# HKU-BAL/MegaGTA

Hardware: AMD Instinct MI355X
Metric: HMM-scored node expansions/sec + SdBG-build Gk-mer/s, k=45, 100Mx150bp (higher is better)
Workload: dtype u32

## Files before the change

include/megagta_hip.h:

```cpp
#ifndef MEGAGTA_HIP_H_
#define MEGAGTA_HIP_H_
#include <stdint.h>
#ifdef __cplusplus
extern "C" {
#endif

#define MGTA_OK 0
#define MGTA_EINVAL (-1)
#define MGTA_EHIP (-2)
#define MGTA_ENOMEM (-3)
#define MGTA_EUNSUPPORTED (-4)
#define MGTA_ESINK (-5)
#define MGTA_EOVERFLOW (-6)
#define MGTA_EINTERNAL (-7)

#define MGTA_NUM_BUCKETS 65536

typedef struct mgta_ctx mgta_ctx;
typedef struct mgta_reads mgta_reads;
typedef struct mgta_sdbg mgta_sdbg;
typedef struct mgta_hmm mgta_hmm;

const char *mgta_last_error(void);
const char *mgta_version(void);
// ... 28 lines not shown

typedef struct mgta_build_stats {
    int32_t k, words_per_key, words_per_tip, n_passes;
    int64_t n_reads, n_kmers;
    int64_t n_items;
    int64_t n_edges, n_tips, n_large;
    int64_t n_sort_launches;
    double ms_total;
    double ms_count, ms_gen, ms_sort, ms_emit, ms_d2h;
    double ms_sort_scatter;
    double ms_local_sort;
    int64_t n_big_segments;
    int64_t n_lsd_tiles;
    uint64_t bytes_peak;
    double ms_stage1;
} mgta_build_stats;

int mgta_reads_upload(mgta_ctx *, const uint32_t *packed_seq, uint64_t n_words, const uint64_t *start_idx,
                      uint64_t n_reads, mgta_reads **out);
int mgta_reads_adopt_device(mgta_ctx *, const uint32_t *d_packed_seq, uint64_t n_words,
                            const uint64_t *d_start_idx, uint64_t n_reads, mgta_reads **out);
void mgta_reads_free(mgta_reads *);

int mgta_sdbg_build_resident(mgta_ctx *, const mgta_reads *, uint64_t n_short_reads, int k, int min_count,
                             int need_mercy, int32_t bucket_begin, int32_t bucket_end ,
                             mgta_edge_sink sink, void *user, mgta_build_stats *stats);
int mgta_sdbg_last_counting(mgta_ctx *, int64_t *hist );
int mgta_sdbg_export_records_device(mgta_ctx *, void *d_dst, uint64_t capacity_bytes, uint64_t *n_records);
int mgta_sdbg_build(mgta_ctx *, const uint32_t *packed_seq, uint64_t n_words, const uint64_t *start_idx,
                    uint64_t n_reads, uint64_t n_short_reads, int k, int min_count, int need_mercy,
// ... 255 lines not shown
```

megagta_amd/_lib.py:

```python
from __future__ import annotations

import ctypes as C
import os

_HERE = os.path.dirname(os.path.abspath(__file__))
LIB_PATH = os.environ.get("MEGAGTA_HIP_LIB") or os.path.join(_HERE, "libmegagta_hip.so")


class MegaGtaError(RuntimeError):
    pass


class DenovoStats(C.Structure):
    _fields_ = [("n_tips", C.c_int64), ("n_bubbles", C.c_int64), ("n_bubble_candidates", C.c_int64), ("n_bubble_rounds", C.c_int64),
                ("n_paths", C.c_int64), ("n_unitig_sweeps", C.c_int64), ("n_contigs", C.c_int64), ("total_len", C.c_int64),
                ("ms_tips", C.c_float), ("ms_bubbles", C.c_float), ("ms_unitigs", C.c_float)]

    def as_dict(self):
        return {n: getattr(self, n) for n, _ in self._fields_}


class BuildStats(C.Structure):
    _fields_ = [("k", C.c_int32), ("words_per_key", C.c_int32), ("words_per_tip", C.c_int32), ("n_passes", C.c_int32),
                ("n_reads", C.c_int64), ("n_kmers", C.c_int64), ("n_items", C.c_int64), ("n_edges", C.c_int64),
                ("n_tips", C.c_int64), ("n_large", C.c_int64), ("n_sort_launches", C.c_int64), ("ms_total", C.c_double),
                ("ms_count", C.c_double), ("ms_gen", C.c_double), ("ms_sort", C.c_double), ("ms_emit", C.c_double),
                ("ms_d2h", C.c_double), ("ms_sort_scatter", C.c_double), ("ms_local_sort", C.c_double), ("n_big_segments", C.c_int64), ("n_lsd_tiles", C.c_int64),
                ("bytes_peak", C.c_uint64), ("ms_stage1", C.c_double)]

    def as_dict(self):
        return {n: getattr(self, n) for n, _ in self._fields_}


class AstarSide(C.Structure):
    _fields_ = [("ok", C.c_int32), ("fval", C.c_int32), ("length", C.c_int32), ("state_no", C.c_int32), ("state", C.c_int32),
                ("partial", C.c_int32), ("node_id", C.c_int64), ("n_closed", C.c_int64), ("n_expanded", C.c_int64),
                ("n_opened", C.c_int64), ("real_score", C.c_double), ("score", C.c_double)]


class AstarStats(C.Structure):
    _fields_ = [("n_seeds", C.c_int64), ("n_expansions", C.c_int64), ("n_opened", C.c_int64), ("n_retries", C.c_int64),
                ("ms_total", C.c_double), ("ms_kernel", C.c_double), ("n_grown", C.c_int64), ("n_rehash", C.c_int64),
                ("n_recycled", C.c_int64), ("pool_bytes", C.c_uint64), ("pool_used", C.c_uint64), ("n_resumes", C.c_int64),
# ... 228 lines not shown
```

megagta_amd/csrc/common.hpp:

```cpp
#pragma once
#include <hip/hip_runtime.h>

#include <cstdarg>
#include <cstdint>
#include <cstdio>
#include <cstring>
#include <exception>
#include <new>
#include <string>
#include <vector>

#include "../../include/megagta_hip.h"

namespace mgta {

void set_error(const char *fmt, ...);

struct HipError {
    int code;
};

#define MGTA_HIP_CHECK(expr)                                                                        \
    do {                                                                                            \
        hipError_t e_ = (expr);                                                                     \
// ... 44 lines not shown
    Timer(Timer &&o) noexcept : a(o.a), b(o.b), st(o.st) { o.a = o.b = nullptr; }
    ~Timer() { if (a) (void)hipEventDestroy(a); if (b) (void)hipEventDestroy(b); }
    void start() { MGTA_HIP_CHECK(hipEventRecord(a, st)); }
    void end() { MGTA_HIP_CHECK(hipEventRecord(b, st)); }
    float ms() const { float t = 0; MGTA_HIP_CHECK(hipEventElapsedTime(&t, a, b)); return t; }
    double stop() {
        MGTA_HIP_CHECK(hipGetLastError());
        end();
        MGTA_HIP_CHECK(hipEventSynchronize(b));
        MGTA_HIP_CHECK(hipGetLastError());
        return ms();
    }
};

enum Slot { S_BLOCK_COUNT, S_BLOCK_BASE, S_SCAN_TMP, S_SMALL, S_KEYS_A, S_KEYS_B, S_HIST, S_TILE_HEADS, S_TILE_BASE, S_CNT, S_BASE,
            S_FIRST, S_OUT_REC, S_OUT_LARGE, S_OUT_TIPS, S_PLAN, S_BIG, S_LSD, S_MULTI_COUNT, S_POS2ID, S_SOLID, S_MERCY, S_EDGE_COUNT, S_SIDE, S_NUM };

}

namespace mgta {
struct AstarArenas {
    DevBuf pool, meta;
};
}

struct mgta_ctx {
    int refs = 1;
    int device = 0;
    hipStream_t stream = nullptr;
    uint64_t mem_limit = 0;
    int force_full_lsd = 0;
// ... 71 lines not shown
```

megagta_amd/csrc/sdbg_build.hip:

```cpp
#include <algorithm>
#include <cmath>
#include <cstdlib>
#include <memory>
#include <type_traits>

#include "common.hpp"
#include "device_utils.hpp"
#include "scan.hpp"

namespace mgta {

constexpr int kDollar = 4;

template <int W>
struct Key {
    uint32_t w[W];
};

template <int W>
__device__ __forceinline__ void shl_bits(uint32_t (&x)[W], int s) {
    if (s == 0) return;
    if (s == 32) {
#pragma unroll
        for (int j = 0; j < W - 1; ++j) x[j] = x[j + 1];
// ... 45 lines not shown
    int k;
    uint32_t b_lo, b_hi;
    uint32_t *block_count;
    const uint64_t *block_base;
    void *out;
    unsigned long long *n_kmers;
    const unsigned long long *is_solid;
    int num_k1_per_read;
    uint64_t n_short;
    unsigned long long *n_sentinel;
    uint32_t multi_width, multi_n;
    uint64_t multi_magic;
    uint8_t *side;
    int side_shift;
    uint32_t side_bias;
};
constexpr int kMaxCountRanges = 64;

template <int W>
__device__ __forceinline__ void keep_masks(int n, uint32_t (&m)[W]) {
#pragma unroll
    for (int j = 0; j < W; ++j) {
        const int lo = j * 16;
        m[j] = n <= lo ? 0u : (n < lo + 16 ? ~0u << (32 - 2 * (n - lo)) : ~0u);
    }
}

template <int W, bool WRITE>
__global__ __launch_bounds__(kScanBlock) void item_scan_kernel(ScanArgs a) {
    __shared__ uint32_t s_cursor;
    __shared__ uint32_t s_wave_cnt[kScanBlock / 64];
    __shared__ uint32_t s_range_cnt[kMaxCountRanges];
    const int k = a.k;
    const int lane = lane_id(), wv = wave_id();
    __shared__ uint64_t s_start[kReadsPerBlock + 1];
    const bool multi = !WRITE && a.multi_n > 0;
    const uint64_t multi_magic = a.multi_magic;
    const bool magic24 = multi_magic < (1u << 24);
    uint64_t r0 = (uint64_t)blockIdx.x * kReadsPerBlock;
    uint64_t r1 = r0 + kReadsPerBlock < a.n_reads ? r0 + kReadsPerBlock : a.n_reads;
    if (threadIdx.x == 0) s_cursor = 0;
    if (!WRITE && threadIdx.x < kMaxCountRanges) s_range_cnt[threadIdx.x] = 0;
    if (threadIdx.x <= r1 - r0) s_start[threadIdx.x] = a.start[r0 + threadIdx.x];
    __syncthreads();
    Key<W> *out = reinterpret_cast<Key<W> *>(a.out);
    uint64_t base = WRITE ? a.block_base[blockIdx.x] : 0;
    uint32_t my_count = 0;
    unsigned long long kmers = 0;
    const int pad_bits = 2 * (16 * W - (k + 1));
    const bool even = !((k + 1) & 1);
    const bool few = multi && a.multi_n <= 8;
    uint32_t acc[8] = {0, 0, 0, 0, 0, 0, 0, 0};
    uint32_t m_edge[W], m_k[W], m_k1[W];
    keep_masks<W>(k + 1, m_edge);
    keep_masks<W>(k, m_k);
    keep_masks<W>(k - 1, m_k1);
    const bool in_bounds = wave_uniform((s_start[r1 - r0] >> 4) + (uint64_t)(W + 1)) < a.n_words;

    auto positions = [&](bool active, uint64_t r, uint64_t s0, int p, int npos) {
        bool run_first = p == 0, run_last = p == npos - 1;
        if (active && a.is_solid && r < a.n_short) {
// ... 21 lines not shown
                for (int j = 0; j <= W; ++j) raw[j] = a.packed[wi + j];
            } else {
#pragma unroll
                for (int j = 0; j <= W; ++j) raw[j] = (wi + j < a.n_words) ? a.packed[wi + j] : 0u;
            }
#pragma unroll
            for (int j = 0; j < W; ++j) e[j] = (uint32_t)(((((uint64_t)raw[j]) << 32) | (uint64_t)raw[j + 1]) >> (32 - sh)) & m_edge[j];
#pragma unroll
            for (int j = 0; j < W; ++j) rc[j] = rev_chars(~e[W - 1 - j]);
            shl_bits<W>(rc, pad_bits);
            bool pal = even;
            if (even) {
#pragma unroll
                for (int j = 0; j < W; ++j) pal = pal && (e[j] == rc[j]);
            }
            auto push = [&](int t, const uint32_t (&src)[W], int from) {
                const uint32_t b = ((src[0] << (2 * from)) >> 16);
                if (b < a.b_lo || b >= a.b_hi) return;
                if (WRITE) mask |= 1u << t;
                else if (multi) {
                    const uint32_t x = b - a.b_lo;
                    uint32_t range;
                    if (magic24) asm("v_mul_hi_u32_u24 %0, %1, %2" : "=v"(range) : "v"(x), "v"((uint32_t)multi_magic));
                    else range = (uint32_t)(((uint64_t)x * multi_magic) >> 32);
                    if (few) fields += 1u << (4 * range);
                    else atomicAdd(&s_range_cnt[range], 1u);
                }
                ++cnt;
            };
            if (run_first) {
                push(0, e, 0);
                if (!pal) push(1, rc, 2);
            }
            push(2, e, 1);
            if (!pal) push(3, rc, 1);
            if (run_last) {
                push(4, e, 2);
                if (!pal) push(5, rc, 0);
            }
        }
        if (!WRITE) {
            my_count += (uint32_t)cnt;
            if (few) {
#pragma unroll
                for (int g = 0; g < 8; ++g)
                    if (g < (int)a.multi_n) acc[g] += (fields >> (4 * g)) & 15u;
            }
        } else {
            const uint32_t inc = wave_incl_scan((uint32_t)cnt);
            const uint32_t tot = __shfl(inc, 63, 64);
            if (tot) {
                uint32_t wbase = 0;
                if (lane == 0) wbase = atomicAdd(&s_cursor, tot);
                const uint64_t first = base + (uint64_t)wave_uniform(wbase);
                char *const wave_out = reinterpret_cast<char *>(out + first);
                uint8_t *const wave_side = a.side ? a.side + first : nullptr;
                uint32_t slot = inc - (uint32_t)cnt;
                auto put = [&](int t, const uint32_t (&src)[W], int from, const uint32_t (&keep)[W], uint32_t flags) {
                    if (!((mask >> t) & 1u)) return;
                    Key<W> key;
#pragma unroll
// ... 52 lines not shown
            for (int g = 0; g < 8; ++g) {
                if (g < (int)a.multi_n) {
                    const uint32_t t = wave_sum(acc[g]);
                    if (lane == 0 && t) atomicAdd(&s_range_cnt[g], t);
                }
            }
        }
        if (lane == 0) s_wave_cnt[wv] = my_count;
        __syncthreads();
        if (threadIdx.x == 0 && !multi) {
            uint32_t t = 0;
            for (int w = 0; w < kScanBlock / 64; ++w) t += s_wave_cnt[w];
            a.block_count[blockIdx.x] = t;
        }
        if (multi && threadIdx.x < a.multi_n) a.block_count[(uint64_t)threadIdx.x * gridDim.x + blockIdx.x] = s_range_cnt[threadIdx.x];
        if (lane == 0 && kmers && a.n_kmers) atomicAdd(a.n_kmers, kmers);
    }
}

template <int W>
__global__ __launch_bounds__(kScanBlock) void item_write_closed_kernel(ScanArgs a) {
    __shared__ uint32_t s_read_base[kReadsPerBlock];
    __shared__ uint64_t s_start[kReadsPerBlock + 1];
    const int k = a.k;
    const int lane = lane_id(), wv = wave_id();
    const uint64_t r0 = (uint64_t)blockIdx.x * kReadsPerBlock;
    const uint64_t r1 = r0 + kReadsPerBlock < a.n_reads ? r0 + kReadsPerBlock : a.n_reads;
    if (wv == 0) {
        const uint64_t st = r0 + lane <= r1 ? a.start[r0 + lane] : 0, st_next = r0 + lane < r1 ? a.start[r0 + lane + 1] : st;
        s_start[lane] = st;
// ... 116 lines not shown
    for (int i = 0; i < N; ++i) { lo[i] = 0; hi[i] = 0; }
#pragma unroll
    for (int j = 0; j < W; ++j) {
        if (j == wi) {
#pragma unroll
            for (int i = 0; i < N; ++i) {
                lo[i] = key[i].w[j] - (BIASED && j == 0 ? d.bias : 0u);
                hi[i] = j > 0 ? key[i].w[j - 1] - (BIASED && j == 1 ? d.bias : 0u) : 0u;
                asm volatile("" : "+v"(lo[i]), "+v"(hi[i]));
            }
        }
    }
    const uint32_t mask = (1u << d.bits) - 1u;
#pragma unroll
    for (int i = 0; i < N; ++i) dg[i] = __builtin_amdgcn_alignbit(hi[i], lo[i], (uint32_t)off) & mask;
}

__device__ __forceinline__ uint32_t xcd_tile(uint32_t b, uint32_t n) {
    if (n < 64) return b;
    const uint32_t x = b & 7u, idx = b >> 3, q = n >> 3, r = n & 7u;
    return x * q + (x < r ? x : r) + idx;
}

template <int W>
__global__ __launch_bounds__(kSortThreads) void radix_census_kernel(const Key<W> *keys, uint64_t n, Digit d, uint64_t n_tiles,
                                                                     uint64_t *hist) {
    __shared__ uint32_t h[256];
    for (int i = threadIdx.x; i < 256; i += kSortThreads) h[i] = 0;
    __syncthreads();
    const uint32_t tile = xcd_tile(blockIdx.x, (uint32_t)n_tiles);
    uint64_t base = (uint64_t)tile * kBlockTile;
    int wi = W - 1 - (d.pos >> 5), off = d.pos & 31;
    bool straddle = off + d.bits > 32 && wi > 0;
    uint32_t mask = (1u << d.bits) - 1u;
    for (int i = 0; i < kBlockTile / kSortThreads; ++i) {
        uint64_t idx = base + (uint64_t)i * kSortThreads + threadIdx.x;
// ... 139 lines not shown
    __shared__ uint64_t carry_s;
    uint64_t *row = hist + (uint64_t)blockIdx.x * n_tiles;
    if (threadIdx.x == 0) carry_s = 0;
    __syncthreads();
    for (uint64_t b = 0; b < n_tiles; b += 1024) {
        uint64_t idx = b + threadIdx.x;
        uint64_t x = idx < n_tiles ? row[idx] : 0, tot;
        uint64_t ex = block_excl_scan64<1024>(x, scratch, &tot);
        uint64_t carry = carry_s;
        if (idx < n_tiles) row[idx] = carry + ex;
        __syncthreads();
        if (threadIdx.x == 0) carry_s = carry + tot;
        __syncthreads();
    }
    if (threadIdx.x == 0) totals[blockIdx.x] = carry_s;
}

template <int W> struct ScatterCfg {
    static constexpr int kIpt = W >= 10 ? 2 : kItemsPerThread;
    static constexpr int kSub = kSortThreads * kIpt;
    static constexpr int kChunk = kSub / kSortWaves;
};

template <int W>
struct ScatterShared {
    Key<W> keys[ScatterCfg<W>::kSub];
    uint16_t whist[kSortWaves][256];
    uint64_t gbase[256];
    uint64_t gdelta[256];
    uint32_t scratch[kSortThreads / 64 + 1];
// ... 928 lines not shown
    if ((int)ctx->pool.size() < S_NUM) ctx->pool.resize(S_NUM);
    DevBuf &b = ctx->pool[slot];
    if (b.bytes < bytes || !b.p) {
        b.release();
        b.alloc(bytes + bytes / 8, &ctx->live_bytes, &ctx->peak_bytes);
    }
    return b.as<T>();
}
static uint64_t pool_bytes(const mgta_ctx *ctx) {
    uint64_t t = 0;
    for (const DevBuf &b : ctx->pool) t += b.bytes;
    return t;
}

struct SortModes {
    int bias = 1, side = 1;
    static SortModes from_env() {
        const char *bias = getenv("MGTA_SORT_BIAS"), *side = getenv("MGTA_SORT_SIDE");
        return SortModes{bias ? atoi(bias) : 1, side ? atoi(side) : 1};
    }
};

static double avg_segment_len(uint64_t n_items, int p, double prefix_frac) { return (double)n_items / std::max(1.0, std::pow(256.0, p) * prefix_frac); }
struct TopPlan {
    int P = 0, skip = 0;
    uint32_t bias = 0;
    double frac = 1.0;
    int T() const { return 8 * P + skip; }
    Digit pass_digit(int W, int i) const { return Digit{32 * W - 8 * (i + 1) - skip, 8, bias}; }
};
static TopPlan choose_top_plan(const mgta_ctx *ctx, uint64_t n_items, int max_top, double prefix_frac, uint32_t b_lo = 0, uint32_t b_hi = 0,
                               int mode = 0) {
    TopPlan plain;
    plain.frac = prefix_frac;
// ... 12 lines not shown
        break;
    }
    return plain;
}

template <int WT>
struct SortJob {
    Key<WT> *a = nullptr, *b = nullptr;
    uint64_t n = 0;
    TopPlan top;
    std::vector<Digit> low;
    uint32_t mask_last2 = ~0u, mask_last = ~0u;
    int side_mode = 1;
    bool census_done = false;
    bool side_done = false;
    bool uses_side() const { return side_mode > 0 && top.P >= 2 && kSideFits<WT>; }
};
struct SortLog {
    mgta_build_stats *S = nullptr;
    std::vector<Timer> scatter;
};

template <int WT>
static Key<WT> *global_passes(mgta_ctx *ctx, const SortJob<WT> &job, SortLog *log) {
    hipStream_t stream = ctx->stream;
    const uint64_t n = job.n, tiles = (n + kBlockTile - 1) / kBlockTile;
    uint64_t *d_hist = pool_get<uint64_t>(ctx, S_HIST, std::max<uint64_t>(1, tiles) * 256 * 8);
    uint64_t *d_totals = pool_get<uint64_t>(ctx, S_SMALL, 4096) + 8;
    uint8_t *d_side = job.uses_side() ? pool_get<uint8_t>(ctx, S_SIDE, n + 64) : nullptr;
    bool side_valid = job.side_done && d_side;
    const dim3 grid((unsigned)tiles), block(kSortThreads);
    Key<WT> *src = job.a, *dst = job.b;
    for (int i = job.top.P - 1; i >= 0; --i) {
        const bool first = i == job.top.P - 1;
        const Digit dg = job.top.pass_digit(WT, i), dn = i > 0 ? job.top.pass_digit(WT, i - 1) : Digit{0, 0, 0};
        if (!(first && job.census_done)) {
            if (side_valid) {
                hipLaunchKernelGGL(radix_census_side_kernel, grid, block, 0, stream, d_side, n, tiles, d_hist);
                if (job.side_mode >= 2) {
                    std::vector<uint64_t> h_side(tiles * 256), h_keys(tiles * 256);
                    MGTA_HIP_CHECK(hipStreamSynchronize(stream));
                    MGTA_HIP_CHECK(hipMemcpy(h_side.data(), d_hist, tiles * 256 * 8, hipMemcpyDeviceToHost));
                    hipLaunchKernelGGL((radix_census_kernel<WT>), grid, block, 0, stream, src, n, dg, tiles, d_hist);
                    MGTA_HIP_CHECK(hipStreamSynchronize(stream));
                    MGTA_HIP_CHECK(hipMemcpy(h_keys.data(), d_hist, tiles * 256 * 8, hipMemcpyDeviceToHost));
                    if (h_side != h_keys) { set_error("internal: side-digit census differs from the census of the keys"); return nullptr; }
                }
            } else
// ... 233 lines not shown
        }
    }
    *is_solid_out = d_solid;
    *num_k1_out = num_k1;
    return MGTA_OK;
}

struct Pass {
    uint32_t b_lo = 0, b_hi = 0, width = 0;
    bool closed_form = false;
    uint64_t n_items = 0, n_tiles = 0, key_b = 0;
    uint64_t n_edges = 0, n_large = 0, n_tips = 0;
    uint16_t *rec = nullptr, *large = nullptr;
    uint32_t *tips = nullptr;
    int64_t *first = nullptr;
    uint32_t nb() const { return b_hi - b_lo; }
};

template <int W>
struct Build {
    mgta_ctx *ctx;
    hipStream_t stream = ctx->stream;
    const mgta_reads *rd = nullptr;
    uint64_t n_short = 0, n_blocks = 0;
    int k = 0, words_per_tip = 0, min_count = 1, need_mercy = 0;
    uint32_t bucket_begin = 0, bucket_end = 0;
    mgta_edge_sink sink = nullptr; void *user = nullptr;
    SortModes modes;
    uint64_t budget = 0;
    bool acc = false;
    ScanArgs sa{};
    uint64_t *d_block_base = nullptr, *d_total = nullptr, *d_kmers = nullptr, *d_tot3 = nullptr, *d_sentinel = nullptr;
    uint32_t multi_n = 0, multi_width = 0, multi_lo = 0;
    uint32_t *d_multi_count = nullptr;
    mgta_build_stats S{};
    Timer t_all{stream}, t_ph{stream};
    SortLog log{&S, {}};
    std::vector<int64_t> h_first, h_items;
    std::vector<uint16_t> h_rec, h_large;
    std::vector<uint32_t> h_tips;
    explicit Build(mgta_ctx *c) : ctx(c) {}

    int run() {
        int rc = start();
        if (rc == MGTA_OK) rc = solid_from_stage1();
        if (rc != MGTA_OK) return rc;
        t_all.start();
        int n_pass = 1;
        for (uint32_t b_lo = bucket_begin; b_lo < bucket_end;) {
            Pass p;
            p.width = (bucket_end - bucket_begin + n_pass - 1) / n_pass;
            p.b_lo = b_lo; p.b_hi = std::min<uint32_t>(bucket_end, b_lo + p.width);
            count_pass(p);
            if (const int more = admit_pass(p, n_pass)) { n_pass = more; continue; }
            S.n_items += (int64_t)p.n_items;
            S.n_passes++;
            if (p.n_items > 0) {
                Key<W> *a = pool_get<Key<W>>(ctx, S_KEYS_A, p.key_b), *b = pool_get<Key<W>>(ctx, S_KEYS_B, p.key_b);
                const SortJob<W> job = plan_sort(p, a, b);
                write_keys(p, job);
                Key<W> *sorted = sort_keys(job);
                if (!sorted) return MGTA_EUNSUPPORTED;
                if ((rc = drop_sentinels(p)) != MGTA_OK || (rc = emit(p, sorted, sorted == a ? b : a)) != MGTA_OK) return rc;
            }
            publish_last(p.b_lo, p.b_hi, p.rec, p.n_edges, p.tips, p.n_tips, p.first, p.large, p.n_large);
            if (acc && p.n_items > 0) append_to_stream(p);
            S.n_edges += (int64_t)p.n_edges; S.n_large += (int64_t)p.n_large; S.n_tips += (int64_t)p.n_tips;
            if ((rc = deliver_pass(p)) != MGTA_OK) return rc;
            b_lo = p.b_hi;
        }
        if (acc) publish_last(bucket_begin, bucket_end, ctx->acc_rec.p, ctx->acc_n_rec, ctx->acc_tips.p, ctx->acc_n_tips, nullptr,
                              ctx->acc_has_large ? ctx->acc_large.p : nullptr, ctx->acc_n_large);
        ctx->acc_valid = acc;
        S.ms_total = t_all.stop();
        for (const Timer &t : log.scatter) S.ms_sort_scatter += t.ms();
        S.bytes_peak = ctx->peak_bytes;
        return MGTA_OK;
    }

    int start() {
        words_per_tip = (2 * k + 31) / 32;
        n_blocks = (rd->n_reads + kReadsPerBlock - 1) / kReadsPerBlock;
        if (n_blocks * (uint64_t)kScanBlock >= (1ull << 32)) { set_error("too many reads for one launch (%llu)", (unsigned long long)rd->n_reads); return MGTA_EUNSUPPORTED; }
        S.k = k; S.words_per_key = W; S.words_per_tip = words_per_tip; S.n_reads = (int64_t)rd->n_reads;
        ctx->peak_bytes = ctx->live_bytes;
        size_t free_b = 0, total_b = 0;
        MGTA_HIP_CHECK(hipMemGetInfo(&free_b, &total_b));
        const uint64_t avail = (uint64_t)free_b + pool_bytes(ctx);
        budget = ctx->mem_limit ? std::min<uint64_t>(ctx->mem_limit, avail) : (uint64_t)(avail * 0.9);
        acc = ctx->keep_stream != 0;
        ctx->acc_valid = false; ctx->acc_n_rec = 0; ctx->acc_n_tips = 0;
        ctx->acc_n_large = 0; ctx->acc_has_large = acc && ctx->keep_multiplicity;
        if (acc) ctx->acc_items.assign(MGTA_NUM_BUCKETS, 0);
        point_scans_at_pool();
        uint64_t *d_small = pool_get<uint64_t>(ctx, S_SMALL, 4096);
        d_total = d_small; d_kmers = d_small + 1; d_tot3 = d_small + 2; d_sentinel = d_small + 5;
        sa.packed = rd->d_packed; sa.n_words = rd->n_words; sa.start = rd->d_start; sa.n_reads = rd->n_reads; sa.k = k; sa.n_short = n_short;
        sa.n_kmers = (unsigned long long *)d_kmers; sa.n_sentinel = (unsigned long long *)d_sentinel;
        return MGTA_OK;
    }
    void point_scans_at_pool() {
        sa.block_count = pool_get<uint32_t>(ctx, S_BLOCK_COUNT, std::max<uint64_t>(1, n_blocks) * 4);
        sa.block_base = d_block_base = pool_get<uint64_t>(ctx, S_BLOCK_BASE, std::max<uint64_t>(1, n_blocks) * 8);
    }

    int solid_from_stage1() {
        if (min_count <= 1) return MGTA_OK;
        unsigned long long *sol = nullptr;
        int nk1 = 0;
        t_ph.start();
        const int rc = run_stage1<W>(ctx, rd, n_short, k, min_count, need_mercy, budget, modes.side, &sol, &nk1);
// ... 6 lines not shown

    void count_pass(Pass &p) {
        const bool first_pass = S.n_passes == 0;
        t_ph.start();
        sa.b_lo = p.b_lo; sa.b_hi = p.b_hi;
        sa.n_kmers = first_pass ? (unsigned long long *)d_kmers : nullptr;
        if (first_pass) MGTA_HIP_CHECK(hipMemsetAsync(d_kmers, 0, 8, stream));
        uint64_t *d_scan_tmp = pool_get<uint64_t>(ctx, S_SCAN_TMP, scan_tmp_elems(std::max<uint64_t>(n_blocks, 1024)) * 8);
        static_assert(kReadsPerBlock == 64, "item_count_closed_kernel: one lane per read of a workgroup");
        p.closed_form = !sa.is_solid && p.b_lo == 0 && p.b_hi == (uint32_t)MGTA_NUM_BUCKETS && !ctx->force_full_lsd;
        const uint32_t *counts = sa.block_count;
        sa.multi_n = 0; sa.multi_width = 0; sa.multi_magic = 0;
        if (n_blocks && (p.closed_form || sa.n_kmers))
            hipLaunchKernelGGL(item_count_closed_kernel, dim3((unsigned)((n_blocks + 63) / 64)), dim3(256), 0, stream, sa.start, sa.n_reads, n_blocks, k,
                               p.closed_form ? sa.block_count : nullptr, sa.n_kmers);
        if (n_blocks && !p.closed_form) {
            sa.n_kmers = nullptr;
            const uint32_t width = p.width, b_lo = p.b_lo, ranges_left = (bucket_end - b_lo + width - 1) / width;
            if (multi_n && (width != multi_width || b_lo < multi_lo || (b_lo - multi_lo) % width != 0 || (b_lo - multi_lo) / width >= multi_n)) multi_n = 0;
            if (!multi_n && ranges_left > 1 && ranges_left <= (uint32_t)kMaxCountRanges) {
                d_multi_count = pool_get<uint32_t>(ctx, S_MULTI_COUNT, (uint64_t)ranges_left * n_blocks * 4);
                ScanArgs sm = sa;
                sm.block_count = d_multi_count; sm.b_hi = bucket_end; sm.multi_width = width; sm.multi_n = ranges_left; sm.multi_magic = ((1ull << 32) + width - 1) / width;
                hipLaunchKernelGGL((item_scan_kernel<W, false>), dim3((unsigned)n_blocks), dim3(kScanBlock), 0, stream, sm);
                multi_n = ranges_left; multi_width = width; multi_lo = b_lo;
            }
            if (multi_n) counts = d_multi_count + (uint64_t)((b_lo - multi_lo) / width) * n_blocks;
            else hipLaunchKernelGGL((item_scan_kernel<W, false>), dim3((unsigned)n_blocks), dim3(kScanBlock), 0, stream, sa);
        }
        exclusive_scan_u32(stream, counts, n_blocks, d_block_base, d_scan_tmp, d_total);
        MGTA_HIP_CHECK(hipMemcpyAsync(&p.n_items, d_total, 8, hipMemcpyDeviceToHost, stream));
        S.ms_count += t_ph.stop();
        if (first_pass) {
            unsigned long long km = 0;
            MGTA_HIP_CHECK(hipMemcpy(&km, d_kmers, 8, hipMemcpyDeviceToHost));
            S.n_kmers = (int64_t)km;
        }
    }

    int admit_pass(Pass &p, int n_pass) {
        p.n_tiles = (p.n_items + kBlockTile - 1) / kBlockTile;
        p.key_b = std::max<uint64_t>(p.n_items * sizeof(Key<W>), p.n_items * 12) + 4096;
        const uint64_t need = 2 * p.key_b + p.n_tiles * 256 * 8 + p.n_items * 2 + p.n_items  + (8u << 20);
        uint64_t other = ctx->live_bytes - pool_bytes(ctx);
        if (acc) {
            const double range_frac = (double)(bucket_end - bucket_begin) / (double)MGTA_NUM_BUCKETS;
            const uint64_t est = (uint64_t)((double)S.n_kmers * 1.5 * range_frac) + (64ull << 20);
            const uint64_t have = ctx->acc_rec.bytes + ctx->acc_tips.bytes;
            other += est > have ? est - have : 0;
        }
        const uint64_t avail = budget - std::min<uint64_t>(budget, other);
        if (need + need / 8 <= avail || p.width <= 1) return 0;
        const double ratio = (double)(need + need / 8) / (double)std::max<uint64_t>(avail, 1) * 1.03;
        return std::max(n_pass + 1, (int)std::ceil((double)n_pass * ratio));
    }

    SortJob<W> plan_sort(const Pass &p, Key<W> *a, Key<W> *b) const {
        const int max_top = (2 * k + 4 + 7) / 8 > 1 ? std::min(4, (32 * W - 8) / 8) : 0;
        SortJob<W> job{a, b, p.n_items, choose_top_plan(ctx, p.n_items, max_top, (double)p.nb() / MGTA_NUM_BUCKETS, p.b_lo, p.b_hi, modes.bias)};
        job.low = low_digit_plan(k, W, job.top.T());
        job.side_mode = modes.side;
        job.census_done = p.closed_form && job.top.P >= 1 && p.n_tiles <= 0x7FFFFFFFull;
        job.side_done = !p.closed_form && job.uses_side();
        return job;
    }

    void write_keys(const Pass &p, const SortJob<W> &job) {
        t_ph.start();
        sa.out = job.a;
        if (p.closed_form) MGTA_HIP_CHECK(hipMemsetAsync(d_sentinel, 0, 8, stream));
        const int shift = 32 - job.top.T();
        if (job.census_done) {
            uint64_t *d_hist = pool_get<uint64_t>(ctx, S_HIST, std::max<uint64_t>(1, p.n_tiles) * 256 * 8);
            hipLaunchKernelGGL((item_write_tiled_kernel<W>), dim3((unsigned)p.n_tiles), dim3(kScanBlock), 0, stream, sa, n_blocks, p.n_items,
                               shift, p.n_tiles, d_hist);
        } else if (p.closed_form)
            hipLaunchKernelGGL((item_write_closed_kernel<W>), dim3((unsigned)n_blocks), dim3(kScanBlock), 0, stream, sa);
        else {
            if (job.side_done) {
                sa.side = pool_get<uint8_t>(ctx, S_SIDE, p.n_items + 64);
                sa.side_shift = shift;
                sa.side_bias = job.top.bias;
            }
            hipLaunchKernelGGL((item_scan_kernel<W, true>), dim3((unsigned)n_blocks), dim3(kScanBlock), 0, stream, sa);
            sa.side = nullptr;
        }
        S.ms_gen += t_ph.stop();
    }

    Key<W> *sort_keys(const SortJob<W> &job) {
        t_ph.start();
        Key<W> *sorted = device_sort(ctx, job, &log);
        if (sorted) S.ms_sort += t_ph.stop();
        return sorted;
    }

    int drop_sentinels(Pass &p) {
        if (!p.closed_form || ((k + 1) & 1)) return MGTA_OK;
        unsigned long long n_sent = 0;
        MGTA_HIP_CHECK(hipMemcpy(&n_sent, d_sentinel, 8, hipMemcpyDeviceToHost));
        if (n_sent >= p.n_items) { set_error("internal: %llu sentinel keys among %llu items", n_sent, (unsigned long long)p.n_items); return MGTA_EINTERNAL; }
        p.n_items -= n_sent;
// ... 253 lines not shown
```

Before: 8.688.

## Fuse first radix sort pass into key writer using per-block census from count scan

The count scan now also builds a per-block 256-bin histogram of the first sort digit. A row scan and a base scan turn that histogram into bin offsets, and the key-writing scan scatters keys straight into their top-digit bins. The radix sort then skips its first pass, which removes one full read and write of the key array plus a separate histogram. In exchange there is extra LDS and atomics in the scan kernels, census memory that may not fit the budget, a plan-mismatch fallback, and an optional validation mode.

```diff
diff --git a/include/megagta_hip.h b/include/megagta_hip.h
--- a/include/megagta_hip.h
+++ b/include/megagta_hip.h
@@ -66,6 +66,8 @@
     int64_t n_lsd_tiles;
     uint64_t bytes_peak;
     double ms_stage1;
+    int64_t n_fused_passes;
+    double ms_fused_write;
 } mgta_build_stats;
 
 int mgta_reads_upload(mgta_ctx *, const uint32_t *packed_seq, uint64_t n_words, const uint64_t *start_idx,
diff --git a/megagta_amd/_lib.py b/megagta_amd/_lib.py
--- a/megagta_amd/_lib.py
+++ b/megagta_amd/_lib.py
@@ -26,7 +26,7 @@
                 ("n_tips", C.c_int64), ("n_large", C.c_int64), ("n_sort_launches", C.c_int64), ("ms_total", C.c_double),
                 ("ms_count", C.c_double), ("ms_gen", C.c_double), ("ms_sort", C.c_double), ("ms_emit", C.c_double),
                 ("ms_d2h", C.c_double), ("ms_sort_scatter", C.c_double), ("ms_local_sort", C.c_double), ("n_big_segments", C.c_int64), ("n_lsd_tiles", C.c_int64),
-                ("bytes_peak", C.c_uint64), ("ms_stage1", C.c_double)]
+                ("bytes_peak", C.c_uint64), ("ms_stage1", C.c_double), ("n_fused_passes", C.c_int64), ("ms_fused_write", C.c_double)]
 
     def as_dict(self):
         return {n: getattr(self, n) for n, _ in self._fields_}
diff --git a/megagta_amd/csrc/common.hpp b/megagta_amd/csrc/common.hpp
--- a/megagta_amd/csrc/common.hpp
+++ b/megagta_amd/csrc/common.hpp
@@ -82,7 +82,7 @@
 };
 
 enum Slot { S_BLOCK_COUNT, S_BLOCK_BASE, S_SCAN_TMP, S_SMALL, S_KEYS_A, S_KEYS_B, S_HIST, S_TILE_HEADS, S_TILE_BASE, S_CNT, S_BASE,
-            S_FIRST, S_OUT_REC, S_OUT_LARGE, S_OUT_TIPS, S_PLAN, S_BIG, S_LSD, S_MULTI_COUNT, S_POS2ID, S_SOLID, S_MERCY, S_EDGE_COUNT, S_SIDE, S_NUM };
+            S_FIRST, S_OUT_REC, S_OUT_LARGE, S_OUT_TIPS, S_PLAN, S_BIG, S_LSD, S_MULTI_COUNT, S_POS2ID, S_SOLID, S_MERCY, S_EDGE_COUNT, S_SIDE, S_CENSUS, S_CENSUS_BASE, S_NUM };
 
 }
 
diff --git a/megagta_amd/csrc/sdbg_build.hip b/megagta_amd/csrc/sdbg_build.hip
--- a/megagta_amd/csrc/sdbg_build.hip
+++ b/megagta_amd/csrc/sdbg_build.hip
@@ -83,8 +83,31 @@
     uint8_t *side;
     int side_shift;
     uint32_t side_bias;
+    uint32_t *census;
+    const uint64_t *row_base;
+    const uint64_t *bin_start;
+    uint64_t out_cap;
+    uint32_t *fuse_error;
+    int cen_shift[8];
+    uint32_t cen_bias[8];
 };
 constexpr int kMaxCountRanges = 64;
+constexpr int kCensusRanges = 8;
+constexpr int kCensusHead = 272;
+constexpr int kCensusRows = 1024;
+
+__device__ __forceinline__ uint32_t xcd_tile(uint32_t b, uint32_t n) {
+    if (n < 64) return b;
+    const uint32_t x = b & 7u, idx = b >> 3, q = n >> 3, r = n & 7u;
+    return x * q + (x < r ? x : r) + idx;
+}
+
+template <int W>
+__device__ __forceinline__ uint32_t item_word0(const uint32_t (&src)[W], int from, uint32_t keep0, uint32_t flags) {
+    const uint32_t nx = W > 1 ? src[W > 1 ? 1 : 0] : 0u;
+    const uint32_t w0 = (from ? ((src[0] << (2 * from)) | (nx >> (32 - 2 * from))) : src[0]) & keep0;
+    return W == 1 ? w0 | flags : w0;
+}
 
 template <int W>
 __device__ __forceinline__ void keep_masks(int n, uint32_t (&m)[W]) {
@@ -95,9 +118,12 @@
     }
 }
 
-template <int W, bool WRITE>
+template <int W, bool WRITE, bool FUSED = false>
 __global__ __launch_bounds__(kScanBlock) void item_scan_kernel(ScanArgs a) {
     __shared__ uint32_t s_cursor;
+    __shared__ uint32_t s_hist[FUSED ? (WRITE ? 256 : kCensusRanges * 256) : 1];
+    __shared__ uint64_t s_bin[FUSED && WRITE ? 256 : 1];
+    __shared__ uint32_t s_cen[FUSED && !WRITE ? 2 * kCensusRanges : 1];
     __shared__ uint32_t s_wave_cnt[kScanBlock / 64];
     __shared__ uint32_t s_range_cnt[kMaxCountRanges];
     const int k = a.k;
@@ -106,14 +132,25 @@
     const bool multi = !WRITE && a.multi_n > 0;
     const uint64_t multi_magic = a.multi_magic;
     const bool magic24 = multi_magic < (1u << 24);
-    uint64_t r0 = (uint64_t)blockIdx.x * kReadsPerBlock;
+    const uint32_t blk = FUSED && WRITE ? xcd_tile(blockIdx.x, gridDim.x) : blockIdx.x;
+    uint64_t r0 = (uint64_t)blk * kReadsPerBlock;
     uint64_t r1 = r0 + kReadsPerBlock < a.n_reads ? r0 + kReadsPerBlock : a.n_reads;
     if (threadIdx.x == 0) s_cursor = 0;
     if (!WRITE && threadIdx.x < kMaxCountRanges) s_range_cnt[threadIdx.x] = 0;
     if (threadIdx.x <= r1 - r0) s_start[threadIdx.x] = a.start[r0 + threadIdx.x];
+    if constexpr (FUSED && WRITE) {
+        static_assert(kScanBlock == 256, "one thread per bin");
+        s_hist[threadIdx.x] = 0;
+        s_bin[threadIdx.x] = a.bin_start[threadIdx.x] + a.row_base[(uint64_t)(blk / kCensusRows) * 256 + threadIdx.x] +
+                             (uint64_t)a.census[(uint64_t)blk * 256 + threadIdx.x];
+    }
+    if constexpr (FUSED && !WRITE) {
+        for (int i = threadIdx.x; i < kCensusRanges * 256; i += kScanBlock) s_hist[i] = 0;
+        if (threadIdx.x < kCensusRanges) { s_cen[2 * threadIdx.x] = (uint32_t)a.cen_shift[threadIdx.x]; s_cen[2 * threadIdx.x + 1] = a.cen_bias[threadIdx.x]; }
+    }
     __syncthreads();
     Key<W> *out = reinterpret_cast<Key<W> *>(a.out);
-    uint64_t base = WRITE ? a.block_base[blockIdx.x] : 0;
+    uint64_t base = WRITE && !FUSED ? a.block_base[blockIdx.x] : 0;
     uint32_t my_count = 0;
     unsigned long long kmers = 0;
     const int pad_bits = 2 * (16 * W - (k + 1));
@@ -165,29 +202,36 @@
 #pragma unroll
                 for (int j = 0; j < W; ++j) pal = pal && (e[j] == rc[j]);
             }
-            auto push = [&](int t, const uint32_t (&src)[W], int from) {
+            auto push = [&](int t, const uint32_t (&src)[W], int from, uint32_t keep0, uint32_t flags) {
                 const uint32_t b = ((src[0] << (2 * from)) >> 16);
                 if (b < a.b_lo || b >= a.b_hi) return;
+                uint32_t range = 0;
                 if (WRITE) mask |= 1u << t;
                 else if (multi) {
                     const uint32_t x = b - a.b_lo;
-                    uint32_t range;
                     if (magic24) asm("v_mul_hi_u32_u24 %0, %1, %2" : "=v"(range) : "v"(x), "v"((uint32_t)multi_magic));
                     else range = (uint32_t)(((uint64_t)x * multi_magic) >> 32);
                     if (few) fields += 1u << (4 * range);
                     else atomicAdd(&s_range_cnt[range], 1u);
                 }
+                if constexpr (FUSED && !WRITE) {
+                    if (range < (uint32_t)kCensusRanges) {
+                        const uint32_t w0 = item_word0<W>(src, from, keep0, flags);
+                        atomicAdd(&s_hist[range * 256u + (((w0 - s_cen[2 * range + 1]) >> s_cen[2 * range]) & 255u)], 1u);
+                    }
+                }
                 ++cnt;
             };
+            const uint32_t e0 = e[0] >> 30, e1 = (e[0] >> 28) & 3u, r0c = rc[0] >> 30, r1c = (rc[0] >> 28) & 3u;
             if (run_first) {
-                push(0, e, 0);
-                if (!pal) push(1, rc, 2);
-            }
-            push(2, e, 1);
-            if (!pal) push(3, rc, 1);
+                push(0, e, 0, m_k[0], 8u | (uint32_t)kDollar);
+                if (!pal) push(1, rc, 2, m_k1[0], r1c);
+            }
+            push(2, e, 1, m_k[0], 8u | e0);
+            if (!pal) push(3, rc, 1, m_k[0], 8u | r0c);
             if (run_last) {
-                push(4, e, 2);
-                if (!pal) push(5, rc, 0);
+                push(4, e, 2, m_k1[0], e1);
+                if (!pal) push(5, rc, 0, m_k[0], 8u | (uint32_t)kDollar);
             }
         }
         if (!WRITE) {
@@ -196,6 +240,35 @@
 #pragma unroll
                 for (int g = 0; g < 8; ++g)
                     if (g < (int)a.multi_n) acc[g] += (fields >> (4 * g)) & 15u;
+            }
+        } else if constexpr (FUSED) {
+            if (mask) {
+                const int shift = a.cen_shift[0];
+                const uint32_t bias = a.cen_bias[0];
+                auto put = [&](int t, const uint32_t (&src)[W], int from, const uint32_t (&keep)[W], uint32_t flags) {
+                    if (!((mask >> t) & 1u)) return;
+                    Key<W> key;
+#pragma unroll
+                    for (int j = 0; j < W; ++j) {
+                        const uint32_t nx = j + 1 < W ? src[j + 1 < W ? j + 1 : j] : 0u;
+                        key.w[j] = (from ? ((src[j] << (2 * from)) | (nx >> (32 - 2 * from))) : src[j]) & keep[j];
+                    }
+                    key.w[W - 1] |= flags;
+                    const uint32_t v = (key.w[0] - bias) >> shift, dg = v & 255u;
+                    const uint64_t slot = s_bin[dg] + (uint64_t)atomicAdd(&s_hist[dg], 1u);
+                    if (slot < a.out_cap) {
+                        out[slot] = key;
+                        if (a.side) a.side[slot] = (uint8_t)(v >> 8);
+                    } else
+                        *a.fuse_error = 1u;
+                };
+                const uint32_t e0 = e[0] >> 30, e1 = (e[0] >> 28) & 3u, r0c = rc[0] >> 30, r1c = (rc[0] >> 28) & 3u;
+                put(0, e, 0, m_k, 8u | (uint32_t)kDollar);
+                put(1, rc, 2, m_k1, r1c);
+                put(2, e, 1, m_k, 8u | e0);
+                put(3, rc, 1, m_k, 8u | r0c);
+                put(4, e, 2, m_k1, e1);
+                put(5, rc, 0, m_k, 8u | (uint32_t)kDollar);
             }
         } else {
             const uint32_t inc = wave_incl_scan((uint32_t)cnt);
@@ -278,6 +351,10 @@
             a.block_count[blockIdx.x] = t;
         }
         if (multi && threadIdx.x < a.multi_n) a.block_count[(uint64_t)threadIdx.x * gridDim.x + blockIdx.x] = s_range_cnt[threadIdx.x];
+        if constexpr (FUSED) {
+            const uint32_t n_ranges = multi ? (a.multi_n < (uint32_t)kCensusRanges ? a.multi_n : (uint32_t)kCensusRanges) : 1u;
+            for (uint32_t g = 0; g < n_ranges; ++g) a.census[((uint64_t)g * gridDim.x + blockIdx.x) * 256 + threadIdx.x] = s_hist[g * 256 + threadIdx.x];
+        }
         if (lane == 0 && kmers && a.n_kmers) atomicAdd(a.n_kmers, kmers);
     }
 }
@@ -424,12 +501,6 @@
     const uint32_t mask = (1u << d.bits) - 1u;
 #pragma unroll
     for (int i = 0; i < N; ++i) dg[i] = __builtin_amdgcn_alignbit(hi[i], lo[i], (uint32_t)off) & mask;
-}
-
-__device__ __forceinline__ uint32_t xcd_tile(uint32_t b, uint32_t n) {
-    if (n < 64) return b;
-    const uint32_t x = b & 7u, idx = b >> 3, q = n >> 3, r = n & 7u;
-    return x * q + (x < r ? x : r) + idx;
 }
 
 template <int W>
@@ -599,6 +670,56 @@
         __syncthreads();
     }
     if (threadIdx.x == 0) totals[blockIdx.x] = carry_s;
+}
+
+__global__ __launch_bounds__(256) void census_rowscan_kernel(uint32_t *cen, uint64_t n_rows, uint64_t *block_tot, uint32_t *overflow) {
+    const uint64_t r0 = (uint64_t)blockIdx.x * kCensusRows, r1 = r0 + kCensusRows < n_rows ? r0 + kCensusRows : n_rows;
+    uint64_t run = 0;
+    for (uint64_t r = r0; r < r1; r += 8) {
+        uint32_t v[8];
+#pragma unroll
+        for (int j = 0; j < 8; ++j) v[j] = r + j < r1 ? cen[(r + j) * 256 + threadIdx.x] : 0u;
+#pragma unroll
+        for (int j = 0; j < 8; ++j) {
+            if (r + j < r1) cen[(r + j) * 256 + threadIdx.x] = (uint32_t)run;
+            run += v[j];
+        }
+    }
+    if (run >> 32) atomicOr(overflow, 1u);
+    block_tot[(uint64_t)blockIdx.x * 256 + threadIdx.x] = run;
+}
+
+__global__ __launch_bounds__(256) void census_base_kernel(uint64_t *block_tot, uint64_t n_row_blocks, uint64_t *bin_start) {
+    __shared__ uint64_t scratch[256 / 64 + 1];
+    uint64_t run = 0;
+    for (uint64_t r = 0; r < n_row_blocks; r += 8) {
+        uint64_t v[8];
+#pragma unroll
+        for (int j = 0; j < 8; ++j) v[j] = r + j < n_row_blocks ? block_tot[(r + j) * 256 + threadIdx.x] : 0ull;
+#pragma unroll
+        for (int j = 0; j < 8; ++j) {
+            if (r + j < n_row_blocks) block_tot[(r + j) * 256 + threadIdx.x] = run;
+            run += v[j];
+        }
+    }
+    uint64_t total = 0;
+    const uint64_t ex = block_excl_scan64<256>(run, scratch, &total);
+    bin_start[threadIdx.x] = ex;
+    if (threadIdx.x == 0) bin_start[256] = total;
+}
+
+template <int W>
+__global__ __launch_bounds__(256) void fused_check_kernel(const Key<W> *keys, uint64_t n, int shift, uint32_t bias, const uint64_t *bin_start,
+                                                          unsigned long long *res) {
+    const uint64_t i = (uint64_t)blockIdx.x * 256 + threadIdx.x;
+    if (i >= n) return;
+    const Key<W> key = keys[i];
+    bool ones = true;
+#pragma unroll
+    for (int j = 0; j < W; ++j) ones = ones && key.w[j] == ~0u;
+    const uint32_t dg = ((key.w[0] - bias) >> shift) & 255u;
+    if (ones) atomicAdd(&res[1], 1ull);
+    else if (i < bin_start[dg] || i >= bin_start[dg + 1]) atomicAdd(&res[0], 1ull);
 }
 
 template <int W> struct ScatterCfg {
@@ -1557,10 +1678,10 @@
 }
 
 struct SortModes {
-    int bias = 1, side = 1;
+    int bias = 1, side = 1, fuse = 1;
     static SortModes from_env() {
-        const char *bias = getenv("MGTA_SORT_BIAS"), *side = getenv("MGTA_SORT_SIDE");
-        return SortModes{bias ? atoi(bias) : 1, side ? atoi(side) : 1};
+        const char *bias = getenv("MGTA_SORT_BIAS"), *side = getenv("MGTA_SORT_SIDE"), *fuse = getenv("MGTA_SORT_FUSE");
+        return SortModes{bias ? atoi(bias) : 1, side ? atoi(side) : 1, fuse ? atoi(fuse) : 1};
     }
 };
 
@@ -1603,6 +1724,7 @@
     int side_mode = 1;
     bool census_done = false;
     bool side_done = false;
+    bool first_done = false;
     bool uses_side() const { return side_mode > 0 && top.P >= 2 && kSideFits<WT>; }
 };
 struct SortLog {
@@ -1620,7 +1742,8 @@
     bool side_valid = job.side_done && d_side;
     const dim3 grid((unsigned)tiles), block(kSortThreads);
     Key<WT> *src = job.a, *dst = job.b;
-    for (int i = job.top.P - 1; i >= 0; --i) {
+    if (job.first_done) std::swap(src, dst);
+    for (int i = job.top.P - 1 - (job.first_done ? 1 : 0); i >= 0; --i) {
         const bool first = i == job.top.P - 1;
         const Digit dg = job.top.pass_digit(WT, i), dn = i > 0 ? job.top.pass_digit(WT, i - 1) : Digit{0, 0, 0};
         if (!(first && job.census_done)) {
@@ -1884,6 +2007,8 @@
     uint16_t *rec = nullptr, *large = nullptr;
     uint32_t *tips = nullptr;
     int64_t *first = nullptr;
+    int plan_row = -1;
+    bool fuse = false;
     uint32_t nb() const { return b_hi - b_lo; }
 };
 
@@ -1903,6 +2028,12 @@
     uint64_t *d_block_base = nullptr, *d_total = nullptr, *d_kmers = nullptr, *d_tot3 = nullptr, *d_sentinel = nullptr;
     uint32_t multi_n = 0, multi_width = 0, multi_lo = 0;
     uint32_t *d_multi_count = nullptr;
+    std::vector<TopPlan> scan_plan;
+    uint32_t scan_lo = 0, scan_width = 0, census_rows = 0;
+    uint32_t *d_census = nullptr;
+    uint32_t *d_fuse_flags = nullptr;
+    bool have_kmers = false;
+    std::vector<Timer> fused_timers;
     mgta_build_stats S{};
     Timer t_all{stream}, t_ph{stream};
     SortLog log{&S, {}};
@@ -1928,7 +2059,7 @@
             if (p.n_items > 0) {
                 Key<W> *a = pool_get<Key<W>>(ctx, S_KEYS_A, p.key_b), *b = pool_get<Key<W>>(ctx, S_KEYS_B, p.key_b);
                 const SortJob<W> job = plan_sort(p, a, b);
-                write_keys(p, job);
+                if ((rc = write_keys(p, job)) != MGTA_OK) return rc;
                 Key<W> *sorted = sort_keys(job);
                 if (!sorted) return MGTA_EUNSUPPORTED;
                 if ((rc = drop_sentinels(p)) != MGTA_OK || (rc = emit(p, sorted, sorted == a ? b : a)) != MGTA_OK) return rc;
@@ -1944,6 +2075,7 @@
         ctx->acc_valid = acc;
         S.ms_total = t_all.stop();
         for (const Timer &t : log.scatter) S.ms_sort_scatter += t.ms();
+        for (const Timer &t : fused_timers) { S.ms_fused_write += t.ms(); S.ms_sort_scatter += t.ms(); }
         S.bytes_peak = ctx->peak_bytes;
         return MGTA_OK;
     }
@@ -1965,6 +2097,7 @@
         point_scans_at_pool();
         uint64_t *d_small = pool_get<uint64_t>(ctx, S_SMALL, 4096);
         d_total = d_small; d_kmers = d_small + 1; d_tot3 = d_small + 2; d_sentinel = d_small + 5;
+        d_fuse_flags = reinterpret_cast<uint32_t *>(d_small + 6);
         sa.packed = rd->d_packed; sa.n_words = rd->n_words; sa.start = rd->d_start; sa.n_reads = rd->n_reads; sa.k = k; sa.n_short = n_short;
         sa.n_kmers = (unsigned long long *)d_kmers; sa.n_sentinel = (unsigned long long *)d_sentinel;
         return MGTA_OK;
@@ -2001,23 +2134,71 @@
         if (n_blocks && (p.closed_form || sa.n_kmers))
             hipLaunchKernelGGL(item_count_closed_kernel, dim3((unsigned)((n_blocks + 63) / 64)), dim3(256), 0, stream, sa.start, sa.n_reads, n_blocks, k,
                                p.closed_form ? sa.block_count : nullptr, sa.n_kmers);
+        uint32_t h_overflow = 0;
         if (n_blocks && !p.closed_form) {
+            const bool plan_first = !sa.is_solid;
+            if (plan_first && sa.n_kmers) {
+                unsigned long long km = 0;
+                MGTA_HIP_CHECK(hipMemcpyAsync(&km, d_kmers, 8, hipMemcpyDeviceToHost, stream));
+                MGTA_HIP_CHECK(hipStreamSynchronize(stream));
+                S.n_kmers = (int64_t)km;
+            }
             sa.n_kmers = nullptr;
+            auto scan = [&](ScanArgs &sm, uint32_t b_lo, uint32_t width, uint32_t ranges, bool may_fuse) {
+                scan_plan.clear(); census_rows = 0;
+                if (plan_first) {
+                    bool any = false;
+                    for (uint32_t r = 0; r < ranges; ++r) {
+                        scan_plan.push_back(plan_ahead(b_lo + r * width, std::min<uint64_t>(bucket_end, (uint64_t)b_lo + (uint64_t)(r + 1) * width)));
+                        any = any || scan_plan.back().P >= 1;
+                    }
+                    scan_lo = b_lo; scan_width = width;
+                    if (any && may_fuse && modes.fuse > 0 && ranges <= (uint32_t)kCensusRanges && census_fits(ranges, width)) {
+                        d_census = pool_get<uint32_t>(ctx, S_CENSUS, (uint64_t)ranges * n_blocks * 256 * 4);
+                        sm.census = d_census;
+                        for (uint32_t r = 0; r < ranges; ++r) { sm.cen_shift[r] = (32 - scan_plan[r].T()) & 31; sm.cen_bias[r] = scan_plan[r].bias; }
+                        hipLaunchKernelGGL((item_scan_kernel<W, false, true>), dim3((unsigned)n_blocks), dim3(kScanBlock), 0, stream, sm);
+                        census_rows = ranges;
+                        return;
+                    }
+                }
+                hipLaunchKernelGGL((item_scan_kernel<W, false>), dim3((unsigned)n_blocks), dim3(kScanBlock), 0, stream, sm);
+            };
             const uint32_t width = p.width, b_lo = p.b_lo, ranges_left = (bucket_end - b_lo + width - 1) / width;
             if (multi_n && (width != multi_width || b_lo < multi_lo || (b_lo - multi_lo) % width != 0 || (b_lo - multi_lo) / width >= multi_n)) multi_n = 0;
             if (!multi_n && ranges_left > 1 && ranges_left <= (uint32_t)kMaxCountRanges) {
                 d_multi_count = pool_get<uint32_t>(ctx, S_MULTI_COUNT, (uint64_t)ranges_left * n_blocks * 4);
                 ScanArgs sm = sa;
                 sm.block_count = d_multi_count; sm.b_hi = bucket_end; sm.multi_width = width; sm.multi_n = ranges_left; sm.multi_magic = ((1ull << 32) + width - 1) / width;
-                hipLaunchKernelGGL((item_scan_kernel<W, false>), dim3((unsigned)n_blocks), dim3(kScanBlock), 0, stream, sm);
+                scan(sm, b_lo, width, ranges_left, true);
                 multi_n = ranges_left; multi_width = width; multi_lo = b_lo;
             }
-            if (multi_n) counts = d_multi_count + (uint64_t)((b_lo - multi_lo) / width) * n_blocks;
-            else hipLaunchKernelGGL((item_scan_kernel<W, false>), dim3((unsigned)n_blocks), dim3(kScanBlock), 0, stream, sa);
+            uint32_t row = 0;
+            if (multi_n) {
+                row = (b_lo - multi_lo) / width;
+                counts = d_multi_count + (uint64_t)row * n_blocks;
+            } else {
+                ScanArgs sm = sa;
+                scan(sm, b_lo, width, 1, ranges_left == 1);
+            }
+            if (row < scan_plan.size()) p.plan_row = (int)row;
+            p.fuse = row < census_rows && scan_plan[row].P >= 1;
+            if (p.fuse) {
+                const uint64_t n_rb = (n_blocks + kCensusRows - 1) / kCensusRows;
+                uint64_t *d_bins = pool_get<uint64_t>(ctx, S_CENSUS_BASE, (kCensusHead + n_rb * 256) * 8);
+                MGTA_HIP_CHECK(hipMemsetAsync(d_fuse_flags, 0, 8, stream));
+                hipLaunchKernelGGL(census_rowscan_kernel, dim3((unsigned)n_rb), dim3(256), 0, stream, d_census + (uint64_t)row * n_blocks * 256, n_blocks,
+                                   d_bins + kCensusHead, d_fuse_flags);
+                hipLaunchKernelGGL(census_base_kernel, dim3(1), dim3(256), 0, stream, d_bins + kCensusHead, n_rb, d_bins);
+                MGTA_HIP_CHECK(hipMemcpyAsync(&h_overflow, d_fuse_flags, 4, hipMemcpyDeviceToHost, stream));
+            }
+        } else {
+            scan_plan.clear(); census_rows = 0;
         }
         exclusive_scan_u32(stream, counts, n_blocks, d_block_base, d_scan_tmp, d_total);
         MGTA_HIP_CHECK(hipMemcpyAsync(&p.n_items, d_total, 8, hipMemcpyDeviceToHost, stream));
         S.ms_count += t_ph.stop();
+        if (h_overflow) p.fuse = false;
         if (first_pass) {
             unsigned long long km = 0;
             MGTA_HIP_CHECK(hipMemcpy(&km, d_kmers, 8, hipMemcpyDeviceToHost));
@@ -2025,10 +2206,12 @@
         }
     }
 
-    int admit_pass(Pass &p, int n_pass) {
-        p.n_tiles = (p.n_items + kBlockTile - 1) / kBlockTile;
-        p.key_b = std::max<uint64_t>(p.n_items * sizeof(Key<W>), p.n_items * 12) + 4096;
-        const uint64_t need = 2 * p.key_b + p.n_tiles * 256 * 8 + p.n_items * 2 + p.n_items  + (8u << 20);
+    static uint64_t pass_need(uint64_t n_items) {
+        const uint64_t n_tiles = (n_items + kBlockTile - 1) / kBlockTile;
+        const uint64_t key_b = std::max<uint64_t>(n_items * sizeof(Key<W>), n_items * 12) + 4096;
+        return 2 * key_b + n_tiles * 256 * 8 + n_items * 2 + n_items  + (8u << 20);
+    }
+    uint64_t avail_bytes() const {
         uint64_t other = ctx->live_bytes - pool_bytes(ctx);
         if (acc) {
             const double range_frac = (double)(bucket_end - bucket_begin) / (double)MGTA_NUM_BUCKETS;
@@ -2036,23 +2219,52 @@
             const uint64_t have = ctx->acc_rec.bytes + ctx->acc_tips.bytes;
             other += est > have ? est - have : 0;
         }
-        const uint64_t avail = budget - std::min<uint64_t>(budget, other);
+        return budget - std::min<uint64_t>(budget, other);
+    }
+    uint64_t census_bytes(uint32_t ranges) const {
+        return ranges ? (uint64_t)ranges * n_blocks * 256 * 4 + (kCensusHead + (n_blocks + kCensusRows - 1) / kCensusRows * 256) * 8 : 0;
+    }
+    bool census_fits(uint32_t ranges, uint32_t width) const {
+        const uint64_t need = pass_need(items_ahead(0, width)) + census_bytes(ranges);
+        return need + need / 8 <= avail_bytes();
+    }
+    uint64_t items_ahead(uint32_t lo, uint32_t hi) const { return (uint64_t)(2.0 * (double)S.n_kmers * (double)(hi - lo) / MGTA_NUM_BUCKETS); }
+    int max_top() const { return (2 * k + 4 + 7) / 8 > 1 ? std::min(4, (32 * W - 8) / 8) : 0; }
+    TopPlan plan_ahead(uint32_t lo, uint32_t hi) const {
+        return choose_top_plan(ctx, items_ahead(lo, hi), max_top(), (double)(hi - lo) / MGTA_NUM_BUCKETS, lo, hi, modes.bias);
+    }
+
+    int admit_pass(Pass &p, int n_pass) {
+        p.n_tiles = (p.n_items + kBlockTile - 1) / kBlockTile;
+        p.key_b = std::max<uint64_t>(p.n_items * sizeof(Key<W>), p.n_items * 12) + 4096;
+        const uint64_t need = pass_need(p.n_items), avail = avail_bytes();
+        const uint64_t with_census = need + census_bytes(census_rows);
+        if (with_census + with_census / 8 <= avail) return 0;
+        if (census_rows && (need + need / 8 <= avail || p.width <= 1)) {
+            ctx->pool[S_CENSUS].release(); ctx->pool[S_CENSUS_BASE].release();
+            census_rows = 0; d_census = nullptr; p.fuse = false;
+        }
         if (need + need / 8 <= avail || p.width <= 1) return 0;
         const double ratio = (double)(need + need / 8) / (double)std::max<uint64_t>(avail, 1) * 1.03;
         return std::max(n_pass + 1, (int)std::ceil((double)n_pass * ratio));
     }
 
-    SortJob<W> plan_sort(const Pass &p, Key<W> *a, Key<W> *b) const {
-        const int max_top = (2 * k + 4 + 7) / 8 > 1 ? std::min(4, (32 * W - 8) / 8) : 0;
-        SortJob<W> job{a, b, p.n_items, choose_top_plan(ctx, p.n_items, max_top, (double)p.nb() / MGTA_NUM_BUCKETS, p.b_lo, p.b_hi, modes.bias)};
+    SortJob<W> plan_sort(Pass &p, Key<W> *a, Key<W> *b) const {
+        SortJob<W> job{a, b, p.n_items, choose_top_plan(ctx, p.n_items, max_top(), (double)p.nb() / MGTA_NUM_BUCKETS, p.b_lo, p.b_hi, modes.bias)};
+        if (p.fuse) {
+            const TopPlan &ahead = scan_plan[p.plan_row];
+            if (ahead.P != job.top.P || ahead.skip != job.top.skip || ahead.bias != job.top.bias) p.fuse = false;
+        }
         job.low = low_digit_plan(k, W, job.top.T());
         job.side_mode = modes.side;
+        job.first_done = p.fuse;
         job.census_done = p.closed_form && job.top.P >= 1 && p.n_tiles <= 0x7FFFFFFFull;
         job.side_done = !p.closed_form && job.uses_side();
         return job;
     }
 
-    void write_keys(const Pass &p, const SortJob<W> &job) {
+    int write_keys(const Pass &p, const SortJob<W> &job) {
+        if (job.first_done) return write_keys_fused(p, job);
         t_ph.start();
         sa.out = job.a;
         if (p.closed_form) MGTA_HIP_CHECK(hipMemsetAsync(d_sentinel, 0, 8, stream));
@@ -2073,6 +2285,46 @@
             sa.side = nullptr;
         }
         S.ms_gen += t_ph.stop();
+        return MGTA_OK;
+    }
+
+    int write_keys_fused(const Pass &p, const SortJob<W> &job) {
+        t_ph.start();
+        const bool check = modes.fuse >= 2;
+        uint64_t *d_bins = ctx->pool[S_CENSUS_BASE].as<uint64_t>();
+        ScanArgs sw = sa;
+        sw.out = job.b; sw.out_cap = p.n_items;
+        sw.census = d_census + (uint64_t)p.plan_row * n_blocks * 256;
+        sw.bin_start = d_bins; sw.row_base = d_bins + kCensusHead;
+        sw.fuse_error = d_fuse_flags + 1;
+        sw.cen_shift[0] = 32 - job.top.T(); sw.cen_bias[0] = job.top.bias;
+        if (job.side_done) sw.side = pool_get<uint8_t>(ctx, S_SIDE, p.n_items + 64);
+        if (check) {
+            MGTA_HIP_CHECK(hipMemsetAsync(job.b, 0xFF, p.n_items * sizeof(Key<W>), stream));
+            MGTA_HIP_CHECK(hipMemsetAsync(d_bins + 264, 0, 16, stream));
+        }
+        fused_timers.emplace_back(stream).start();
+        hipLaunchKernelGGL((item_scan_kernel<W, true, true>), dim3((unsigned)n_blocks), dim3(kScanBlock), 0, stream, sw);
+        fused_timers.back().end();
+        uint32_t refused = 0;
+        MGTA_HIP_CHECK(hipMemcpyAsync(&refused, d_fuse_flags + 1, 4, hipMemcpyDeviceToHost, stream));
+        S.ms_gen += t_ph.stop();
+        S.n_sort_launches++; S.n_fused_passes++;
+        if (refused) { set_error("internal: the fused key writer ran past the census of its bins"); return MGTA_EINTERNAL; }
+        if (check) {
+            hipLaunchKernelGGL((fused_check_kernel<W>), dim3((unsigned)((p.n_items + 255) / 256)), dim3(256), 0, stream, job.b, p.n_items, 32 - job.top.T(),
+                               job.top.bias, d_bins, (unsigned long long *)(d_bins + 264));
+            uint64_t res[2] = {0, 0}, total = 0;
+            MGTA_HIP_CHECK(hipMemcpyAsync(res, d_bins + 264, 16, hipMemcpyDeviceToHost, stream));
+            MGTA_HIP_CHECK(hipMemcpyAsync(&total, d_bins + 256, 8, hipMemcpyDeviceToHost, stream));
+            MGTA_HIP_CHECK(hipStreamSynchronize(stream));
+            if (total != p.n_items || res[0] || res[1]) {
+                set_error("internal: fused first pass: census of %llu keys for %llu items, %llu keys outside their bin, %llu slots not written",
+                          (unsigned long long)total, (unsigned long long)p.n_items, (unsigned long long)res[0], (unsigned long long)res[1]);
+                return MGTA_EINTERNAL;
+            }
+        }
+        return MGTA_OK;
     }
 
     Key<W> *sort_keys(const SortJob<W> &job) {
```

New measurement: 7.215. -17.0%, worse.
